# OpenHardware-Initiative/Drone-OA-IREE-ViT-Accelerator

Hardware: AMD Instinct MI355X
Metric: frames/s on ITAViTLSTM int8, 60x90 depth input (higher is better)
Workload: dtype int8+f32; 1 GPU; ITAViTLSTM int8 end-to-end forward (BASELINE config 4): 1024 synthetic 60x90 depth frames per GPU per step, LSTM state carried, velocity all-gather; frames_per_gpu=1024, global_batch=1024, parallelism=dp1, image_dtype=u8, weights=seed-0 synthetic QAT (tests/golden), gather_every=1, gather=none (one GPU), schedule=one stream

## Files before the change

### drone-oa-iree-vit-accelerator_amd/csrc/ita_lstm_head_kernel.h

```cpp
#pragma once
#include <cstddef>
#include "ita_f16x3_kernels.h"

__device__ __forceinline__ size_t ita_lstm_plane_index(int b, int k) {
  return ((size_t)(((b >> 5) * 4 + (k >> 6)) * 4 + ((k >> 4) & 3)) * 64 + ((k >> 3) & 1) * 32 + (b & 31)) * 8 + (k & 7);
}
__device__ __forceinline__ float lstm_sigmoid_fast(float x) {
  return __builtin_amdgcn_rcpf(1.0f + __builtin_amdgcn_exp2f(x * -1.44269504088896341f));
}
__device__ __forceinline__ float lstm_tanh_fast(float x) {
  return 1.0f - 2.0f * __builtin_amdgcn_rcpf(__builtin_amdgcn_exp2f(x * 2.88539008177792681f) + 1.0f);
}

__device__ __forceinline__ f32x16 mfma_f16x3(f32x16 acc, f16x8 wh, f16x8 wl, f16x8 xh, f16x8 xl) {
  acc = __builtin_amdgcn_mfma_f32_32x32x16_f16(wl, xh, acc, 0, 0, 0);
  acc = __builtin_amdgcn_mfma_f32_32x32x16_f16(wh, xl, acc, 0, 0, 0);
  return __builtin_amdgcn_mfma_f32_32x32x16_f16(wh, xh, acc, 0, 0, 0);
}
__device__ __forceinline__ void lstm_cell_fast(float gi, float gf, float gg, float go, float c_prev, float& c, float& h) {
  const float ig = lstm_sigmoid_fast(gi), fg = lstm_sigmoid_fast(gf), cg = lstm_tanh_fast(gg), og = lstm_sigmoid_fast(go);
  c = fmaf(fg, c_prev, ig * cg);
  h = og * lstm_tanh_fast(c);
}
__device__ __forceinline__ void split_f16x4(f32x4 x, f16x4& hi, f16x4& lo) {
#pragma unroll
  for (int j = 0; j < 4; ++j) {
    _Float16 a, b;
    split_f16(x[j], a, b);
    hi[j] = a;
    lo[j] = b;
  }
}
__device__ __forceinline__ f32x4 lstm_l0_extra(float dv, f32x4 q, int h, float& x4) {
  f32x4 x0 = {0.0f, 0.0f, 0.0f, 0.0f};
  x4 = 0.0f;
  if (h == 0) {
    x0 = (f32x4){dv / 10.0f, q.x, q.y, q.z};
    x4 = q.w;
  }
  return x0;
}
template <int NS>
__device__ __forceinline__ f32x4 sum_partials(const f32x4 (&pz)[NS]) {
  f32x4 ps = pz[0];
#pragma unroll
  for (int z = 1; z < NS; ++z) ps += pz[z];
  return ps;
}
__device__ __forceinline__ float lstm_sum4(const float (*part)[16][64], int e, int pl) {
  return ((part[0][e][pl] + part[1][e][pl]) + part[2][e][pl]) + part[3][e][pl];
}
template <class Live>
__device__ __forceinline__ void lstm_fc_rows(const float (*hs)[132], const float (*fw)[128], const float* fc_b, float* vel,
                                             size_t row0, int f0, int B, int tid, Live live) {
  if (tid < 96) {
    const int fr = tid / 3, o = tid - 3 * fr, b = f0 + fr;
    if (b < B && live(b)) {
      float acc = fc_b[o];
      for (int k = 0; k < 128; ++k) acc = fmaf(hs[fr][k], fw[o][k], acc);
      vel[(row0 + b) * 3 + o] = acc;
    }
  }
}

constexpr int ITA_HEAD_CNT_STRIDE = 64;
constexpr unsigned ITA_HEAD_ERR_TIMEOUT = 1;
constexpr unsigned long long ITA_HEAD_SPIN_TICKS = 200000000ull;
__device__ __forceinline__ void ita_store_sc1_f16x4(f16x4 v, __amdgpu_buffer_rsrc_t rsrc, int byte_off) {
  __builtin_amdgcn_raw_buffer_store_b64(__builtin_bit_cast(u32x2, v), rsrc, byte_off, 0, ITA_SC1);
}
__device__ __forceinline__ void ita_gather_h8(float hn, _Float16 (*pub)[32][8], int ef, int eu) {
  _Float16 x, y;
  split_f16(hn, x, y);
  pub[0][ef][eu] = x;
  pub[1][ef][eu] = y;
  __syncthreads();
}
__device__ __forceinline__ void ita_publish_h8(const _Float16 (*pub)[32][8], int r, __amdgpu_buffer_rsrc_t hi, int off_hi,
                                               __amdgpu_buffer_rsrc_t lo, int off_lo) {
  const f16x8 vh = *(const f16x8*)&pub[0][r][0], vl = *(const f16x8*)&pub[1][r][0];
  __builtin_amdgcn_raw_buffer_store_b128(__builtin_bit_cast(u32x4, vh), hi, off_hi, 0, ITA_SC1);
  __builtin_amdgcn_raw_buffer_store_b128(__builtin_bit_cast(u32x4, vl), lo, off_lo, 0, ITA_SC1);
}
__device__ __forceinline__ f16x8 ita_load_sc1_f16x8(__amdgpu_buffer_rsrc_t rsrc, int byte_off) {
  return __builtin_bit_cast(f16x8, __builtin_amdgcn_raw_buffer_load_b128(rsrc, byte_off, 0, ITA_SC1));
}
__device__ __forceinline__ f32x4 ita_load_sc1_f32x4(__amdgpu_buffer_rsrc_t rsrc, int byte_off) {
  return __builtin_bit_cast(f32x4, __builtin_amdgcn_raw_buffer_load_b128(rsrc, byte_off, 0, ITA_SC1));
}
__device__ __forceinline__ unsigned ita_head_arrive(unsigned* cnt, int ft, int tid) {
  asm volatile("s_waitcnt vmcnt(0)" ::: "memory");
  __syncthreads();
  unsigned prev = 0;
  if (tid == 0) prev = __hip_atomic_fetch_add(cnt + ft * ITA_HEAD_CNT_STRIDE, 1u, __ATOMIC_RELAXED, __HIP_MEMORY_SCOPE_AGENT);
// ... 1 lines not shown
}
__device__ __forceinline__ bool ita_head_poll(unsigned* cnt, unsigned target, unsigned* err) {
  const unsigned long long t0 = wall_clock64();
  while (__hip_atomic_load(cnt, __ATOMIC_RELAXED, __HIP_MEMORY_SCOPE_AGENT) < target) {
    if (wall_clock64() - t0 > ITA_HEAD_SPIN_TICKS) {
      __hip_atomic_fetch_or(err, ITA_HEAD_ERR_TIMEOUT, __ATOMIC_RELAXED, __HIP_MEMORY_SCOPE_AGENT);
      return false;
    }
    __builtin_amdgcn_s_sleep(2);
  }
  return true;
}


struct ItaLstmModelArgs {
  const float* part; float inv_fold_scale;
  const _Float16 *w0_hi, *w0_lo; float inv_wscale0;
  const float* bias0;
  const _Float16 *w1_hi, *w1_lo, *w2_hi, *w2_lo;
  float inv_wscale1, inv_wscale2;
  const float *bsum1, *bsum2;
};
struct ItaLstmHeadArgs {
  ItaLstmModelArgs m;
  const float *desvel, *quat;
  const float *h_in, *c_in;
  float *h_out, *c_out;
  size_t lstride;
  _Float16 *p1_hi, *p1_lo, *p2_hi, *p2_lo;
  const float *fc_w, *fc_b; float* vel;
  unsigned *cnt, *err;
  int B;
  const int* slots;
};
static_assert(sizeof(ItaLstmModelArgs) == 104 && offsetof(ItaLstmHeadArgs, desvel) == 104, "kernel-argument layout");

template <int NS>
__global__ __launch_bounds__(256, 2) void ita_lstm_head_kernel(const ItaLstmHeadArgs a) {
  __shared__ __attribute__((aligned(16))) float big[32 * 132 + 32 * 36];
  __shared__ __attribute__((aligned(16))) f16x8 hin[2][2][4][2][64];
  __shared__ __attribute__((aligned(16))) _Float16 pub[2][32][8];
  __shared__ unsigned flag;
  float (*hs)[132] = (float (*)[132])big;
  float (*pt)[36] = (float (*)[36])(big + 32 * 132);
  float (*part)[16][64] = (float (*)[16][64])big;
  const int tid = threadIdx.x, lane = tid & 63, wave = __builtin_amdgcn_readfirstlane(tid >> 6);
  const int ft = blockIdx.x >> 4, ut = blockIdx.x & 15, f0 = ft * 32;
  const int r = lane & 31, h = lane >> 5;
  const int B = a.B;
  const int ef = tid >> 3, eu = tid & 7;
  int rh[4], rb0 = min(f0 + r, B - 1), reb = min(f0 + ef, B - 1);
#pragma unroll
  for (int i = 0; i < 4; ++i) rh[i] = min(f0 + 2 * (4 * wave + i) + h, B - 1);
  if (a.slots) {
#pragma unroll
    for (int i = 0; i < 4; ++i) rh[i] = a.slots[rh[i]];
    rb0 = a.slots[rb0];
    reb = a.slots[reb];
  }

  f32x4 pz[NS];
#pragma unroll
  for (int z = 0; z < NS; ++z)
    pz[z] = *(const f32x4*)(a.m.part + ((size_t)z * B + min(f0 + 8 * wave + (lane >> 3), B - 1)) * 512 + ut * 32 + 4 * (lane & 7));
  f32x4 hv[4];
#pragma unroll
  for (int i = 0; i < 4; ++i) hv[i] = *(const f32x4*)(a.h_in + (size_t)rh[i] * 128 + 4 * r);
  const int b0 = f0 + r, u0 = ut * 8 + 4 * h;
  const size_t sb0 = (size_t)rb0;
  if (wave >= 2) {
    f32x4 hx[2][4][2];
#pragma unroll
    for (int l = 0; l < 2; ++l)
#pragma unroll
      for (int s = 0; s < 4; ++s) {
        const float* src = a.h_in + (l + 1) * a.lstride + sb0 * 128 + 64 * (wave - 2) + 16 * s + 8 * h;
        hx[l][s][0] = *(const f32x4*)src;
        hx[l][s][1] = *(const f32x4*)(src + 4);
      }
    __builtin_amdgcn_sched_barrier(0);
#pragma unroll
    for (int l = 0; l < 2; ++l)
// ... 15 lines not shown
  f32x4 q = {0.0f, 0.0f, 0.0f, 0.0f}, ci0 = {0.0f, 0.0f, 0.0f, 0.0f}, bz[4];
  float dv = 0.0f;
  if (wave == 0) {
    const _Float16* wfr_hi = a.m.w0_hi + ((size_t)ut * 9 * 64 + lane) * 8;
    const _Float16* wfr_lo = a.m.w0_lo + ((size_t)ut * 9 * 64 + lane) * 8;
#pragma unroll
    for (int s = 0; s < 9; ++s) {
      wh[s] = *(const f16x8*)(wfr_hi + s * 512);
      wl[s] = *(const f16x8*)(wfr_lo + s * 512);
    }
    const int bc = min(b0, B - 1);
    q = *(const f32x4*)(a.quat + (size_t)bc * 4);
    dv = a.desvel[bc];
    ci0 = *(const f32x4*)(a.c_in + sb0 * 128 + u0);
#pragma unroll
    for (int gt = 0; gt < 4; ++gt) bz[gt] = *(const f32x4*)(a.m.bias0 + gt * 128 + u0);
  }
  const size_t wo = ((size_t)((ut * 4 + wave) * 4) * 64 + lane) * 8;
  f16x8 w1h[4], w1l[4];
#pragma unroll
  for (int s = 0; s < 4; ++s) {
    w1h[s] = *(const f16x8*)(a.m.w1_hi + wo + 512 * s);
    w1l[s] = *(const f16x8*)(a.m.w1_lo + wo + 512 * s);
  }
  const int eb = f0 + ef, un = ut * 8 + eu;
  const size_t esb = (size_t)reb;
  const float c1_prev = a.c_in[a.lstride + esb * 128 + un], c2_prev = a.c_in[2 * a.lstride + esb * 128 + un];
  float bs1[4], bs2[4];
#pragma unroll
  for (int gt = 0; gt < 4; ++gt) {
    bs1[gt] = a.m.bsum1[gt * 128 + un];
    bs2[gt] = a.m.bsum2[gt * 128 + un];
  }
  __builtin_amdgcn_sched_barrier(0);
  *(f32x4*)&pt[8 * wave + (lane >> 3)][4 * (lane & 7)] = sum_partials(pz);
#pragma unroll
  for (int i = 0; i < 4; ++i) *(f32x4*)&hs[2 * (4 * wave + i) + h][4 * r] = hv[i];
  __syncthreads();

  f32x4 hn0 = {0.0f, 0.0f, 0.0f, 0.0f};
  if (wave == 0) {
    f32x16 acc = {};
    float xlast1;
    const f32x4 xlast0 = lstm_l0_extra(dv, q, h, xlast1);
#pragma unroll
    for (int s = 0; s < 9; ++s) {
      f32x4 x0 = xlast0, x1 = {xlast1, 0.0f, 0.0f, 0.0f};
      if (s < 8) {
        x0 = *(const f32x4*)&hs[r][16 * s + 8 * h];
        x1 = *(const f32x4*)&hs[r][16 * s + 8 * h + 4];
      }
      f16x8 xh, xl;
#pragma unroll
      for (int j = 0; j < 8; ++j) {
        const float x = j < 4 ? x0[j & 3] : x1[j & 3];
        const _Float16 hi = (_Float16)x;
        xh[j] = hi;
        xl[j] = (_Float16)(x - (float)hi);
      }
      acc = mfma_f16x3(acc, wh[s], wl[s], xh, xl);
    }
    f32x4 cn;
#pragma unroll
    for (int q = 0; q < 4; ++q) {
      float g[4];
#pragma unroll
      for (int gt = 0; gt < 4; ++gt)
        g[gt] = (pt[r][gt * 8 + 4 * h + q] * a.m.inv_fold_scale + acc[4 * gt + q] * a.m.inv_wscale0) + bz[gt][q];
      float c, hn;
      lstm_cell_fast(g[0], g[1], g[2], g[3], ci0[q], c, hn);
      cn[q] = c;
      hn0[q] = hn;
    }
    if (b0 < B) *(f32x4*)(a.c_out + sb0 * 128 + u0) = cn;
    f16x4 x_hi, x_lo;
    split_f16x4(hn0, x_hi, x_lo);
    const int o0 = (int)ita_lstm_plane_index(b0, u0) * 2;
    ita_store_sc1_f16x4(x_hi, ita_rsrc(a.p1_hi), o0);
    ita_store_sc1_f16x4(x_lo, ita_rsrc(a.p1_lo), o0);
  }
  (void)ita_head_arrive(a.cnt, ft, tid);
  f16x8 w2h[4], w2l[4];
#pragma unroll
  for (int s = 0; s < 4; ++s) {
    w2h[s] = *(const f16x8*)(a.m.w2_hi + wo + 512 * s);
    w2l[s] = *(const f16x8*)(a.m.w2_lo + wo + 512 * s);
  }

#pragma unroll
  for (int l = 1; l <= 2; ++l) {
    if (tid == 0) flag = ita_head_poll(a.cnt + ft * ITA_HEAD_CNT_STRIDE, 16u * l, a.err) ? 1u : 0u;
    __syncthreads();
    if (!flag) return;
    if (l == 1 && wave == 0 && b0 < B) *(f32x4*)(a.h_out + sb0 * 128 + u0) = hn0;
    f16x8 fah[4], fal[4];
    if (wave < 2) {
      const int ao = (((ft * 4 + wave) * 4) * 64 + lane) * 16;
      const _Float16* ph = l == 1 ? a.p1_hi : a.p2_hi;
      const _Float16* pl = l == 1 ? a.p1_lo : a.p2_lo;
#pragma unroll
      for (int s = 0; s < 4; ++s) {
        fah[s] = ita_load_sc1_f16x8(ita_rsrc(ph), ao + 1024 * s);
        fal[s] = ita_load_sc1_f16x8(ita_rsrc(pl), ao + 1024 * s);
      }
    } else {
#pragma unroll
      for (int s = 0; s < 4; ++s) {
        fah[s] = hin[l - 1][wave - 2][s][0][lane];
        fal[s] = hin[l - 1][wave - 2][s][1][lane];
      }
    }
    f32x16 acc = {};
#pragma unroll
    for (int s = 0; s < 4; ++s) acc = mfma_f16x3(acc, l == 1 ? w1h[s] : w2h[s], l == 1 ? w1l[s] : w2l[s], fah[s], fal[s]);
#pragma unroll
    for (int e = 0; e < 16; ++e) part[wave][e][lane] = acc[e];
    __syncthreads();
    float gsum[4];
    const int pl = ef + 32 * (eu >> 2);
#pragma unroll
    for (int gte = 0; gte < 4; ++gte) gsum[gte] = lstm_sum4(part, 4 * gte + (eu & 3), pl);
    const float iws = l == 1 ? a.m.inv_wscale1 : a.m.inv_wscale2;
    const float* bs = l == 1 ? bs1 : bs2;
    const float gi = gsum[0] * iws + bs[0], gf = gsum[1] * iws + bs[1], gg = gsum[2] * iws + bs[2], go = gsum[3] * iws + bs[3];
    float c, hn;
    lstm_cell_fast(gi, gf, gg, go, l == 1 ? c1_prev : c2_prev, c, hn);
    const size_t so = l * a.lstride + esb * 128 + un;
    if (eb < B) {
      a.c_out[so] = c;
      if (l == 1) a.h_out[so] = hn;
      else
        __builtin_amdgcn_raw_buffer_store_b32(__builtin_bit_cast(unsigned, hn), ita_rsrc(a.h_out), (int)(so * 4), 0, ITA_SC1);
    }
    if (l == 1) {
      ita_gather_h8(hn, pub, ef, eu);
      if (wave == 0 && h == 0) {
        const int o = (int)ita_lstm_plane_index(f0 + r, ut * 8) * 2;
        ita_publish_h8(pub, r, ita_rsrc(a.p2_hi), o, ita_rsrc(a.p2_lo), o);
      }
    }
    const unsigned prev = ita_head_arrive(a.cnt, ft, tid);
    if (tid == 0 && l == 2) flag = prev == 47u ? 1u : 0u;
  }

  __syncthreads();
  if (!flag) return;
  if (tid == 0) __hip_atomic_store(a.cnt + ft * ITA_HEAD_CNT_STRIDE, 0u, __ATOMIC_RELAXED, __HIP_MEMORY_SCOPE_AGENT);
  float (*fw)[128] = (float (*)[128])(big + 32 * 132);
  int fro[4];
#pragma unroll
  for (int i = 0; i < 4; ++i) fro[i] = min(f0 + ((i * 256 + tid) >> 5), B - 1);
  if (a.slots) {
#pragma unroll
    for (int i = 0; i < 4; ++i) fro[i] = a.slots[fro[i]];
  }
  f32x4 hr[4];
#pragma unroll
  for (int i = 0; i < 4; ++i)
    hr[i] = ita_load_sc1_f32x4(ita_rsrc(a.h_out), (int)((2 * a.lstride + (size_t)fro[i] * 128 + 4 * (tid & 31)) * 4));
  const f32x4 wv = *(const f32x4*)(a.fc_w + 4 * min(tid, 95));
#pragma unroll
  for (int i = 0; i < 4; ++i) *(f32x4*)&hs[(i * 256 + tid) >> 5][4 * (tid & 31)] = hr[i];
  if (tid < 96) *(f32x4*)&fw[tid >> 5][4 * (tid & 31)] = wv;
  __syncthreads();
  lstm_fc_rows(hs, fw, a.fc_b, a.vel, 0, f0, B, tid, [](int) { return true; });
}
```

### drone-oa-iree-vit-accelerator_amd/csrc/ita_lstm_seq_kernel.h

```cpp
#pragma once
#include "ita_lstm_head_kernel.h"

constexpr int ITA_SEQ_PLANE = 2 * 4 * 64 * 16;
constexpr int ITA_SEQ_P1 = 0, ITA_SEQ_P2 = 2 * ITA_SEQ_PLANE;
constexpr int ITA_SEQ_H2 = 4 * ITA_SEQ_PLANE;
constexpr int ITA_SEQ_PARITY = ITA_SEQ_H2 + 32 * 128 * 4;
constexpr int ITA_SEQ_TILE = 2 * ITA_SEQ_PARITY;

struct ItaLstmSeqArgs {
  ItaLstmModelArgs m;
  const float *desvel, *quat;
  float *state_h, *state_c;
  const int* lengths; int t0;
  char* ho;
  const float *fc_w, *fc_b; float* vel;
  unsigned *cnt, *err;
  int B, nsteps;
};
static_assert(offsetof(ItaLstmSeqArgs, desvel) == 104, "kernel-argument layout");

__device__ __forceinline__ int ita_seq_plane_off(int r, int k) {
  return ((((k >> 6) * 4 + ((k >> 4) & 3)) * 64 + ((k >> 3) & 1) * 32 + r) * 8 + (k & 7)) * 2;
}

template <int NS>
__global__ __launch_bounds__(256, 1) void ita_lstm_seq_kernel(const ItaLstmSeqArgs a) {
  __shared__ __attribute__((aligned(16))) float big[32 * 132];
  __shared__ __attribute__((aligned(16))) float pt[32][36];
  __shared__ __attribute__((aligned(16))) float fw[3][128];
  __shared__ __attribute__((aligned(16))) _Float16 pub[2][32][8];
  __shared__ __attribute__((aligned(16))) f16x8 w0s[2][9][64];
  __shared__ unsigned flag;
  float (*hs)[132] = (float (*)[132])big;
  float (*acc4)[16][64] = (float (*)[16][64])big;
  const int tid = threadIdx.x, lane = tid & 63, wave = __builtin_amdgcn_readfirstlane(tid >> 6);
  const int ft = blockIdx.x >> 4, ut = blockIdx.x & 15, f0 = ft * 32;
  const int r = lane & 31, h = lane >> 5;
  const int B = a.B;
  unsigned* const cnt = a.cnt + ft * ITA_HEAD_CNT_STRIDE;
  const __amdgpu_buffer_rsrc_t ho = ita_rsrc(a.ho + (size_t)ft * ITA_SEQ_TILE);

  int nt = a.nsteps;
  if (a.lengths) {
    int m = 0;
    for (int i = 0; i < 32; ++i) m = max(m, a.lengths[min(f0 + i, B - 1)]);
    nt = min(nt, max(m - a.t0, 0));
  }
  if (nt <= 0) return;

  const int b0 = f0 + r, u0 = ut * 8 + 4 * h, bc0 = min(b0, B - 1);
  f32x4 c0 = {0.0f, 0.0f, 0.0f, 0.0f}, h0 = {0.0f, 0.0f, 0.0f, 0.0f}, bz[4];
  int len0 = 0;
  if (wave == 0) {
    const _Float16* wfr_hi = a.m.w0_hi + ((size_t)ut * 9 * 64 + lane) * 8;
    const _Float16* wfr_lo = a.m.w0_lo + ((size_t)ut * 9 * 64 + lane) * 8;
#pragma unroll
    for (int s = 0; s < 9; ++s) {
      w0s[0][s][lane] = *(const f16x8*)(wfr_hi + s * 512);
      w0s[1][s][lane] = *(const f16x8*)(wfr_lo + s * 512);
    }
    c0 = *(const f32x4*)(a.state_c + (size_t)bc0 * 128 + u0);
    h0 = *(const f32x4*)(a.state_h + (size_t)bc0 * 128 + u0);
#pragma unroll
    for (int gt = 0; gt < 4; ++gt) bz[gt] = *(const f32x4*)(a.m.bias0 + gt * 128 + u0);
    len0 = b0 < B ? (a.lengths ? a.lengths[b0] - a.t0 : a.nsteps) : 0;
  }
  const size_t wo = ((size_t)((ut * 4 + wave) * 4) * 64 + lane) * 8;
  f16x8 w1h[4], w1l[4], w2h[4], w2l[4];
#pragma unroll
  for (int s = 0; s < 4; ++s) {
    w1h[s] = *(const f16x8*)(a.m.w1_hi + wo + 512 * s);
    w1l[s] = *(const f16x8*)(a.m.w1_lo + wo + 512 * s);
    w2h[s] = *(const f16x8*)(a.m.w2_hi + wo + 512 * s);
    w2l[s] = *(const f16x8*)(a.m.w2_lo + wo + 512 * s);
  }
  const int ef = tid >> 3, eu = tid & 7, eb = f0 + ef, un = ut * 8 + eu, ebc = min(eb, B - 1);
  const size_t lstride = (size_t)B * 128;
  const size_t so1 = lstride + (size_t)ebc * 128 + un, so2 = so1 + lstride;
  float c1 = a.state_c[so1], c2 = a.state_c[so2], h1 = a.state_h[so1], h2 = a.state_h[so2];
  const int lenE = eb < B ? (a.lengths ? a.lengths[eb] - a.t0 : a.nsteps) : 0;
  float bs1[4], bs2[4];
#pragma unroll
  for (int gt = 0; gt < 4; ++gt) {
    bs1[gt] = a.m.bsum1[gt * 128 + un];
    bs2[gt] = a.m.bsum2[gt * 128 + un];
  }
  if (tid < 96) *(f32x4*)&fw[tid >> 5][4 * (tid & 31)] = *(const f32x4*)(a.fc_w + 4 * tid);
  const size_t zstride = (size_t)a.nsteps * B * 512;
  const size_t prow = (size_t)min(f0 + 8 * wave + (lane >> 3), B - 1) * 512 + ut * 32 + 4 * (lane & 7);
  f32x4 ps;
  {
    f32x4 pz[NS];
#pragma unroll
    for (int z = 0; z < NS; ++z) pz[z] = *(const f32x4*)(a.m.part + z * zstride + prow);
    ps = sum_partials(pz);
  }
  f32x4 q = {0.0f, 0.0f, 0.0f, 0.0f};
  float dv = 0.0f;
  if (wave == 0) {
    q = *(const f32x4*)(a.quat + (size_t)bc0 * 4);
    dv = a.desvel[bc0];
  }

  auto publish_h0 = [&](int par) {
    f16x4 x_hi, x_lo;
    split_f16x4(h0, x_hi, x_lo);
    const int o = par * ITA_SEQ_PARITY + ITA_SEQ_P1 + ita_seq_plane_off(r, u0);
    ita_store_sc1_f16x4(x_hi, ho, o);
    ita_store_sc1_f16x4(x_lo, ho, o + ITA_SEQ_PLANE);
  };
  auto publish_h1 = [&](int par) {
    ita_gather_h8(h1, pub, ef, eu);
    if (wave == 0 && h == 0) {
      const int o = par * ITA_SEQ_PARITY + ITA_SEQ_P2 + ita_seq_plane_off(r, ut * 8);
      ita_publish_h8(pub, r, ho, o, ho, o + ITA_SEQ_PLANE);
    }
  };
  auto publish_h2 = [&](int par) {
    __builtin_amdgcn_raw_buffer_store_b32(__builtin_bit_cast(unsigned, h2), ho, par * ITA_SEQ_PARITY + ITA_SEQ_H2 + (ef * 128 + un) * 4,
                                          0, ITA_SC1);
  };
  auto fc_step = [&](int par, int t) {
    f32x4 hr[4];
#pragma unroll
    for (int i = 0; i < 4; ++i)
      hr[i] = ita_load_sc1_f32x4(ho, par * ITA_SEQ_PARITY + ITA_SEQ_H2 + (((i * 256 + tid) >> 5) * 128 + 4 * (tid & 31)) * 4);
#pragma unroll
    for (int i = 0; i < 4; ++i) *(f32x4*)&hs[(i * 256 + tid) >> 5][4 * (tid & 31)] = hr[i];
    __syncthreads();
    lstm_fc_rows(hs, fw, a.fc_b, a.vel, (size_t)t * B, f0, B, tid, [&](int b) { return !a.lengths || a.t0 + t < a.lengths[b]; });
    __syncthreads();
  };

  if (wave == 0) publish_h0(1);
  publish_h1(1);
  publish_h2(1);
  (void)ita_head_arrive(a.cnt, ft, tid);
  if (tid == 0) flag = ita_head_poll(cnt, 16u, a.err) ? 1u : 0u;
  __syncthreads();
  if (!flag) return;

  for (int t = 0; t < nt; ++t) {
    const int par = t & 1, prv = par ^ 1;
    *(f32x4*)&pt[8 * wave + (lane >> 3)][4 * (lane & 7)] = ps;
    f16x8 xh[8], xl[8];
    if (wave == 0) {
#pragma unroll
      for (int s = 0; s < 8; ++s) {
        xh[s] = ita_load_sc1_f16x8(ho, prv * ITA_SEQ_PARITY + ITA_SEQ_P1 + (s * 64 + lane) * 16);
        xl[s] = ita_load_sc1_f16x8(ho, prv * ITA_SEQ_PARITY + ITA_SEQ_P1 + ITA_SEQ_PLANE + (s * 64 + lane) * 16);
      }
    }
    __syncthreads();
    if (wave == 0) {
      f32x16 acc = {};
#pragma unroll
      for (int s = 0; s < 8; ++s) acc = mfma_f16x3(acc, w0s[0][s][lane], w0s[1][s][lane], xh[s], xl[s]);
      {
        float x1;
        const f32x4 x0 = lstm_l0_extra(dv, q, h, x1);
        f16x8 yh, yl;
#pragma unroll
        for (int j = 0; j < 8; ++j) {
          const float x = j < 4 ? x0[j & 3] : (j == 4 ? x1 : 0.0f);
// ... 64 lines not shown
        for (int s = 0; s < 4; ++s)
#pragma unroll
          for (int j = 0; j < 8; ++j) {
            _Float16 hi, lo;
            split_f16(hx[s][j >> 2][j & 3], hi, lo);
            fah[s][j] = hi;
            fal[s][j] = lo;
          }
      }
      f32x16 acc = {};
#pragma unroll
      for (int s = 0; s < 4; ++s) acc = mfma_f16x3(acc, l == 1 ? w1h[s] : w2h[s], l == 1 ? w1l[s] : w2l[s], fah[s], fal[s]);
#pragma unroll
      for (int e = 0; e < 16; ++e) acc4[wave][e][lane] = acc[e];
      __syncthreads();
      float gsum[4];
      const int pl = ef + 32 * (eu >> 2);
#pragma unroll
      for (int gte = 0; gte < 4; ++gte) gsum[gte] = lstm_sum4(acc4, 4 * gte + (eu & 3), pl);
      const float iws = l == 1 ? a.m.inv_wscale1 : a.m.inv_wscale2;
      const float* bs = l == 1 ? bs1 : bs2;
      const float gi = gsum[0] * iws + bs[0], gf = gsum[1] * iws + bs[1], gg = gsum[2] * iws + bs[2], go = gsum[3] * iws + bs[3];
      float c, hn;
      lstm_cell_fast(gi, gf, gg, go, l == 1 ? c1 : c2, c, hn);
      if (t < lenE) {
        if (l == 1) { c1 = c; h1 = hn; }
        else        { c2 = c; h2 = hn; }
      }
      if (l == 1) {
        publish_h1(par);
        (void)ita_head_arrive(a.cnt, ft, tid);
      } else {
        publish_h2(par);
      }
    }
  }

  if (wave == 0 && b0 < B) {
    *(f32x4*)(a.state_c + (size_t)b0 * 128 + u0) = c0;
    *(f32x4*)(a.state_h + (size_t)b0 * 128 + u0) = h0;
  }
  if (eb < B) {
    a.state_c[so1] = c1; a.state_h[so1] = h1;
    a.state_c[so2] = c2; a.state_h[so2] = h2;
  }
  const unsigned prev = ita_head_arrive(a.cnt, ft, tid);
  if (tid == 0) flag = prev == 16u * (2u * nt + 2u) - 1u ? 1u : 0u;
  __syncthreads();
  if (!flag) return;
  if (tid == 0) __hip_atomic_store(cnt, 0u, __ATOMIC_RELAXED, __HIP_MEMORY_SCOPE_AGENT);
  fc_step((nt - 1) & 1, nt - 1);
}
```

### drone-oa-iree-vit-accelerator_amd/csrc/ita_plugin.hip

```cpp
#include <hip/hip_runtime.h>

#include <algorithm>
#include <cstdio>
#include <cstdlib>
#include <cstring>
#include <mutex>
#include <string>
#include <atomic>
#include <thread>
#include <memory>
#include <type_traits>
#include <vector>

#include "../../include/ita_mi355x.h"
#include "../../include/ita_weights.h"
#include "../../include/ita_wire.h"
#include "ita_f16x3_kernels.h"
#include "ita_lstm_head_kernel.h"
#include "ita_lstm_seq_kernel.h"
#include "ita_f32_kernels.h"
#include "ita_int8_kernels.h"
#include "ita_stream_kernel.h"
#include "ita_long_attn_kernel.h"
#include "ita_long_stats_kernel.h"
// ... 86 lines not shown
  operator T*() const { return p; }
};

int launch_tail(int num_cus, int E, const float* wT, const float* bias, const float* x, float* feat, int ld, int B,
                hipStream_t s) {
  if (!wT) return fail(ITA_ERR_BAD_BLOB, "fusion-tail parameters missing from the blob");
  if (E != 64) return fail(ITA_ERR_UNSUPPORTED, "fusion tail is built for E = 64 (ITAViTLSTM)");
  ItaTailArgs a{x, wT, bias, feat, ld, B};
  const int grid = B < 2 * num_cus ? B : 2 * num_cus;
  return launch<ita_tail_kernel<64>, ita_tail_lds_bytes<64>()>(dim3(grid), dim3(256), s, a);
}

int launch_gemm(const float* A, int lda, const float* W, int ldw, const float* bias, float* C, int ldc, int M, int N,
                int K, hipStream_t s) {
  if (N % 64 || K % 32) return fail(ITA_ERR_UNSUPPORTED, "gemm needs N % 64 == 0 and K % 32 == 0");
  ItaGemmArgs g{A, lda, W, ldw, bias, C, ldc, M, N, K};
  return launch<ita_gemm_f32_kernel>(dim3(N / 64, (M + 31) / 32), dim3(256), s, g);
}

}

#include "ita_weights_load.h"

namespace {

struct Workspace {
  int cap = 0;
  int front_cap[ITA_PART_BUFFERS] = {};
  DevBuf<float> bufA, bufB, cat0, cat1, cat2, gates, feat;
  DevBuf<_Float16> x2_hi, x2_lo, c1_hi, c1_lo, c2_hi, c2_lo;
  DevBuf<float> part;
  DevBuf<unsigned> head_sync;
  size_t head_sync_bytes = 0;
  DevBuf<char> seq_ho;
};

struct TailLarge {
  DevBuf<_Float16> hi, lo;
  DevBuf<_Float16> up_hi, up_lo;
  DevBuf<_Float16> ps_hi, ps_lo;
  DevBuf<float> bias;
  float inv_scale = 1.0f;
  int E = 0, CO = 0, nt = 0, nchunk = 0;
};

struct WireSize {
  int H = 0, W = 0;
  DevBuf<int> idx;
  DevBuf<float> coeff;
  ItaWireTables dev{};
  int span[3] = {};
};
constexpr int ITA_WIRE_SIZES = 8;

}

struct ita_context {
  int device = 0;
  int num_cus = 256;
  Weights w;
  Workspace ws;
  bool ws_reserved = false;
  TailLarge tl;
  int tail_mode = 1;
  bool prof = false;
  int prof_max = 0, prof_n = 0;
// ... 15 lines not shown
};

namespace {

std::mutex g_bind_mu;
ita_handle g_bound = nullptr;
int g_bound_layer = 0;
int g_bound_dtype = ITA_DISPATCH_F16;

bool capturing(hipStream_t s) {
  hipStreamCaptureStatus cs = hipStreamCaptureStatusNone;
  return hipStreamIsCapturing(s, &cs) == hipSuccess && cs != hipStreamCaptureStatusNone;
}

int grow_workspace(ita_context* c, int B) {
  c->ws = Workspace{};
  Workspace& ws = c->ws;
  const size_t E = (size_t)c->w.hdr.E, nb = (size_t)B, ntile = (nb + 31) / 32;
  HIPCHK(ws.bufA.alloc(nb * 128 * E));
  HIPCHK(ws.bufB.alloc(nb * 128 * E));
  HIPCHK(ws.feat.alloc(nb * 4608));
  HIPCHK(ws.cat0.alloc(nb * K0P));
  HIPCHK(ws.cat1.alloc(nb * 256));
  HIPCHK(ws.cat2.alloc(nb * 256));
  HIPCHK(ws.gates.alloc(nb * 512));
  HIPCHK(ws.x2_hi.alloc(2 * nb * c->w.ldfold));
  HIPCHK(ws.x2_lo.alloc(2 * nb * c->w.ldfold));
  for (DevBuf<_Float16>* b : {&ws.c1_hi, &ws.c1_lo, &ws.c2_hi, &ws.c2_lo})
    HIPCHK(b->alloc(ntile * 32 * 256));
  HIPCHK(ws.part.alloc(ITA_PART_BUFFERS * (size_t)NSPLIT * nb * 512));
  ws.head_sync_bytes = sizeof(unsigned) * ITA_HEAD_CNT_STRIDE * (1 + ntile);
  HIPCHK(ws.head_sync.alloc(ITA_HEAD_CNT_STRIDE * (1 + ntile)));
  HIPCHK(hipMemset(ws.head_sync, 0, ws.head_sync_bytes));
  HIPCHK(ws.seq_ho.alloc((size_t)ITA_SEQ_TILE * ntile));
  HIPCHK(hipDeviceSynchronize());
  ws.cap = B;
  return ITA_OK;
}

int ensure_workspace(ita_context* c, int B, hipStream_t s) {
  if (B <= c->ws.cap) return ITA_OK;
  if (c->ws_reserved)
    return fail(ITA_ERR_INVALID_ARG, "batch exceeds the workspace pinned by ita_reserve; call ita_reserve(max_batch) again while idle");
  if (capturing(s))
    return fail(ITA_ERR_INVALID_ARG, "the workspace cannot grow inside a stream capture; call ita_reserve first");
  return grow_workspace(c, B);
}

int check(ita_handle h, int batch, bool need_weights = true) {
  if (!h) return fail(ITA_ERR_INVALID_ARG, "null handle");
  if (batch <= 0) return fail(ITA_ERR_INVALID_ARG, "batch must be positive");
  if (need_weights && !h->w.loaded) return fail(ITA_ERR_NO_WEIGHTS, "ita_load_weights has not been called");
  HIPCHK(hipSetDevice(h->device));
  return ITA_OK;
}

int check_layer_io(ita_handle h, int layer, const void* x, const void* y, int batch) {
  if (int rc = check(h, batch)) return rc;
  if (!x || !y || layer < 0 || layer >= h->w.hdr.num_layers) return fail(ITA_ERR_INVALID_ARG, "bad pointer or layer");
  return ITA_OK;
}

ItaMhaArgs mha_args(ita_context* c, int layer, const float* x, float* y, int B, bool fuse, const ita_mha_taps* t) {
  const Layer& L = c->w.layers[layer];
  ItaMhaArgs a{};
  a.x = x; a.y = y;
// ... 983 lines not shown
int ita_get_attn_kind(ita_handle h, int layer, int* kind) {
  if (!h || !h->w.loaded) return fail(ITA_ERR_NO_WEIGHTS, "no weights loaded");
  if (!kind || layer < 0 || layer >= h->w.hdr.num_layers) return fail(ITA_ERR_INVALID_ARG, "bad pointer or layer");
  *kind = h->w.layers[layer].attn_f32 ? ITA_ATTN_F32 : ITA_ATTN_INT8;
  return ITA_OK;
}

int ita_mha_f32(ita_handle h, int layer, const float* x, float* y, int batch, void* stream) {
  if (int rc = check_layer_io(h, layer, x, y, batch)) return rc;
  return launch_attn_f32(h, layer, x, y, batch, false, (hipStream_t)stream);
}

int ita_encoder_layer(ita_handle h, int layer, const float* x, float* y, int batch, void* stream) {
  if (int rc = check_layer_io(h, layer, x, y, batch)) return rc;
  StreamIo io;
  io.x = x; io.y = y;
  return launch_encoder(h, layer, io, batch, (hipStream_t)stream);
}

int ita_debug_encoder_stamps(ita_handle h, int layer, const float* x, const void* image_u8, float* y, int batch,
                             unsigned long long* stamps, void* stream) {
  int rc = check(h, batch);
  if (rc) return rc;
  if ((!x && !image_u8) || !y || !stamps || layer < 0 || layer >= h->w.hdr.num_layers)
    return fail(ITA_ERR_INVALID_ARG, "bad argument");
  if (h->w.layers[layer].attn_f32) return fail(ITA_ERR_UNSUPPORTED, "this layer's attention is float32 (ITAW0003 blob): no stream kernel, no stamps");
  if (image_u8 ? !h->w.layers[layer].simg_tok : !h->w.layers[layer].simg_enc)
    return fail(ITA_ERR_UNSUPPORTED, "this layer does not run on the stream kernel");
  StreamIo io;
  io.x = x; io.y = y; io.stamps = stamps; io.img = image_u8;
  return launch_encoder(h, layer, io, batch, (hipStream_t)stream);
}

#ifdef ITA_UP_STAMP
int ita_debug_tail_up_stamps(unsigned long long* host_dst, int count) {
  if (hipDeviceSynchronize() != hipSuccess) return ITA_ERR_HIP;
  return hipMemcpyFromSymbol(host_dst, HIP_SYMBOL(ita_up_stamp_buf), sizeof(unsigned long long) * (size_t)count) == hipSuccess ? ITA_OK : ITA_ERR_HIP;
}
#endif
int ita_debug_softmax_rows(ita_handle h, const int8_t* logits, uint8_t* probs, int rows, void* stream) {
  int rc = check(h, rows, false);
  if (rc) return rc;
  if (!logits || !probs) return fail(ITA_ERR_INVALID_ARG, "null pointer");
  return launch<ita_softmax_rows_kernel>(dim3((rows + 15) / 16), dim3(64), (hipStream_t)stream, logits, probs, rows);
}

int ita_debug_fast_site_ok(float mult) { return fast_site_ok(mult) ? 1 : 0; }
int ita_debug_fused_site(float mult, int* C, float* K) {
  if (!C || !K) return 0;
  return fused_site(mult, ITA_MAGIC128_F, ITA_FUSED_DMAX, C, K) ? 1 : 0;
}
int ita_debug_fused_check(float mult, int form, int C, float* K) {
  float k = 0.0f;
  const int ok = fused_site_check(mult, form == 1 ? ITA_MAGIC32K_F : form == 2 ? ITA_MAGIC_F : ITA_MAGIC128_F, C, &k) ? 1 : 0;
  if (K) *K = k;
  return ok;
}
int ita_debug_layer_fused(ita_handle h, int layer, unsigned* fused_sites, int* fused, int* C6, float* K6) {
  if (!h || !h->w.loaded) return fail(ITA_ERR_NO_WEIGHTS, "no weights loaded");
  if (!fused_sites || !fused || layer < 0 || layer >= h->w.hdr.num_layers)
    return fail(ITA_ERR_INVALID_ARG, "ita_debug_layer_fused: null output or layer out of range");
  const Layer& L = h->w.layers[layer];
  *fused_sites = L.fused_sites;
  *fused = L.fused ? (L.fused_relu ? 2 : 1) : 0;
  for (int i = 0; i < 6; ++i) {
    if (C6) C6[i] = L.fused_c[i];
// ... 213 lines not shown
      return true;
    };
    if (span_ok(tok_h, OH, 16, ItaTailUpLds::RH) && span_ok(tok_w, OW, 32, ItaTailUpLds::RW)) {
      ItaTailUpArgs u{x, h->tl.up_hi, h->tl.up_lo, h->tl.ps_hi, h->tl.ps_lo, h->tl.bias, h->tl.inv_scale, out, batch, tok_h, tok_w, h->tl.CO};
      const long ntiles = (long)(OW / 32) * (OH / 16) * batch;
      return launch<ita_tail_up_kernel, ItaTailUpLds::TOTAL>(dim3((unsigned)(ntiles < h->num_cus ? ntiles : h->num_cus)), dim3(512), s, u);
    }
  }
  switch (h->tl.nt) {
    case 1: return launch_tail_big<1>(a, s);
    case 2: return launch_tail_big<2>(a, s);
    case 3: return launch_tail_big<3>(a, s);
    default: return launch_tail_big<4>(a, s);
  }
}

static ItaLstmModelArgs lstm_model_args(const ita_context* h, const float* part) {
  const auto& w = h->w;
  ItaLstmModelArgs m;
  m.part = part;          m.inv_fold_scale = w.fold_inv_scale;
  m.w0_hi = w.lw_hi[0];   m.w0_lo = w.lw_lo[0];   m.inv_wscale0 = w.lw_inv_scale[0];
  m.bias0 = w.fold_bias;
  m.w1_hi = w.lw_hi[1];   m.w1_lo = w.lw_lo[1];   m.inv_wscale1 = w.lw_inv_scale[1];
  m.w2_hi = w.lw_hi[2];   m.w2_lo = w.lw_lo[2];   m.inv_wscale2 = w.lw_inv_scale[2];
  m.bsum1 = w.bsum[1];    m.bsum2 = w.bsum[2];
  return m;
}
static dim3 lstm_grid(int B) { return dim3(16 * ((B + 31) / 32)); }

static int launch_lstm_head(ita_context* h, const float* part, const float* desvel, const float* quat, const float* h_in,
                            const float* c_in, float* h_out, float* c_out, size_t lstride, float* vel, int B,
                            const int* slots, hipStream_t s) {
  ItaLstmHeadArgs p{lstm_model_args(h, part), desvel, quat, h_in, c_in, h_out, c_out, lstride,
                    h->ws.c1_hi, h->ws.c1_lo, h->ws.c2_hi, h->ws.c2_lo, h->w.fc_w, h->w.fc_b, vel, h->ws.head_sync + ITA_HEAD_CNT_STRIDE, h->ws.head_sync, B, slots};
  return launch<ita_lstm_head_kernel<NSPLIT>>(lstm_grid(B), dim3(256), s, p);
}

static int launch_lstm_seq(ita_context* h, const float* desvel, const float* quat, float* state_h, float* state_c,
                           const int* lengths, int t0, float* vel, int B, int n, hipStream_t s) {
  ItaLstmSeqArgs p{lstm_model_args(h, h->ws.part), desvel, quat, state_h, state_c, lengths, t0, h->ws.seq_ho,
                   h->w.fc_w, h->w.fc_b, vel, h->ws.head_sync + ITA_HEAD_CNT_STRIDE, h->ws.head_sync, B, n};
  return launch<ita_lstm_seq_kernel<NSPLIT>>(lstm_grid(B), dim3(256), s, p);
}

static int forward_impl(ita_handle h, const void* image, int image_dtype, const float* desvel, const float* quat,
                        const float* h_in, const float* c_in, float* vel, float* h_out, float* c_out, int batch,
                        const ita_forward_taps* taps, void* stream, const int* slots, int state_rows,
                        const float* x2_in = nullptr) {
  int rc = check(h, batch);
  if (rc) return rc;
  if ((!image && !x2_in) || !desvel || !quat || !h_in || !c_in || !vel || !h_out || !c_out)
    return fail(ITA_ERR_INVALID_ARG, "null pointer");
  if (image_dtype != ITA_IMAGE_F32 && image_dtype != ITA_IMAGE_U8) return fail(ITA_ERR_INVALID_ARG, "bad image dtype");
  if (!h->w.dec_w || !h->w.wcat[0] || !h->w.fc_w || (h->w.hdr.has_tail && !h->w.tail_wT))
    return fail(ITA_ERR_BAD_BLOB, "blob holds no decoder / LSTM (/ fusion tail) parameters");
  if (h->w.hdr.has_tail && h->w.hdr.E != 64) return fail(ITA_ERR_UNSUPPORTED, "the fusion tail is built for E = 64 (ITAViTLSTM)");
  if ((rc = ensure_workspace(h, batch, (hipStream_t)stream))) return rc;
  hipStream_t s = (hipStream_t)stream;
  const int B = batch;
  const size_t tokb = sizeof(float) * (size_t)B * 128 * h->w.hdr.E;
  const bool fast = h->tail_mode == 1 && h->w.folded;
  if (slots && !fast) return fail(ITA_ERR_UNSUPPORTED, "slot-indexed state needs tail mode 1");
  const size_t lstride = (size_t)(slots ? state_rows : batch) * 128;
  StageRecorder rec(h, s, true);
  if ((rc = rec.mark())) return rc;
  const bool fused_tok = !x2_in && fuse_tokenizer(h, image_dtype);
  if (slots && !x2_in) {
    const Layer& LL = h->w.layers.back();
// ... 383 lines not shown
```

Baseline: 11.29 million frames/s.

## Distribute final FC head across unit-tile blocks via partial sums

Each of the 16 unit-tile workgroups now computes a 3-output partial dot product over its own 8 hidden units of the last LSTM layer. It publishes these partials to a new fc_part buffer. The last-arriving workgroup then only sums 16 partials per output, instead of reloading the full 32x128 h tile and fc weights and running a 128-long dot product. The sequence kernel gets the same treatment, and optional timestamp instrumentation is added behind a compile flag. This trades an extra small global store per block and a shared barrier for removing the serial tail reload and compute.

```diff
diff --git a/drone-oa-iree-vit-accelerator_amd/csrc/ita_lstm_head_kernel.h b/drone-oa-iree-vit-accelerator_amd/csrc/ita_lstm_head_kernel.h
--- a/drone-oa-iree-vit-accelerator_amd/csrc/ita_lstm_head_kernel.h
+++ b/drone-oa-iree-vit-accelerator_amd/csrc/ita_lstm_head_kernel.h
@@ -50,16 +50,51 @@
 __device__ __forceinline__ float lstm_sum4(const float (*part)[16][64], int e, int pl) {
   return ((part[0][e][pl] + part[1][e][pl]) + part[2][e][pl]) + part[3][e][pl];
 }
+constexpr int ITA_FC_PART_TILE = 16 * 32 * 4;
+__device__ __forceinline__ f32x4 lstm_fc_partial(const float (*hf)[8], int fr, const float (&fcw)[3][8]) {
+  const f32x4 h0 = *(const f32x4*)&hf[fr][0], h1 = *(const f32x4*)&hf[fr][4];
+  f32x4 p = {0.0f, 0.0f, 0.0f, 0.0f};
+#pragma unroll
+  for (int o = 0; o < 3; ++o) {
+    float s = 0.0f;
+#pragma unroll
+    for (int u = 0; u < 8; ++u) s = fmaf(u < 4 ? h0[u & 3] : h1[u & 3], fcw[o][u], s);
+    p[o] = s;
+  }
+  return p;
+}
 template <class Live>
-__device__ __forceinline__ void lstm_fc_rows(const float (*hs)[132], const float (*fw)[128], const float* fc_b, float* vel,
-                                             size_t row0, int f0, int B, int tid, Live live) {
+__device__ __forceinline__ void lstm_fc_sum(__amdgpu_buffer_rsrc_t fp, int byte_off, const float* fc_b, float* vel, size_t row0,
+                                            int f0, int B, int tid, Live live) {
   if (tid < 96) {
     const int fr = tid / 3, o = tid - 3 * fr, b = f0 + fr;
+    float p[16];
+#pragma unroll
+    for (int ut = 0; ut < 16; ++ut)
+      p[ut] = __builtin_bit_cast(float, __builtin_amdgcn_raw_buffer_load_b32(fp, byte_off + ((ut * 32 + fr) * 4 + o) * 4, 0, ITA_SC1));
     if (b < B && live(b)) {
       float acc = fc_b[o];
-      for (int k = 0; k < 128; ++k) acc = fmaf(hs[fr][k], fw[o][k], acc);
+#pragma unroll
+      for (int ut = 0; ut < 16; ++ut) acc += p[ut];
       vel[(row0 + b) * 3 + o] = acc;
     }
+  }
+}
+constexpr int ITA_HEAD_STAMPS = 12, ITA_HEAD_STAMP_WGS = 1024;
+#ifdef ITA_HEAD_STAMP
+__device__ unsigned long long ita_head_stamp_buf[ITA_HEAD_STAMP_WGS * ITA_HEAD_STAMPS];
+constexpr bool ITA_HEAD_STAMPED = true;
+__device__ __forceinline__ void ita_head_stamp_put(int wg, int i) {
+  if (wg < ITA_HEAD_STAMP_WGS) ita_head_stamp_buf[wg * ITA_HEAD_STAMPS + i] = wall_clock64();
+}
+#else
+constexpr bool ITA_HEAD_STAMPED = false;
+__device__ __forceinline__ void ita_head_stamp_put(int, int) {}
+#endif
+template <bool STAMP>
+__device__ __forceinline__ void ita_head_stamp(int i) {
+  if constexpr (STAMP) {
+    if (threadIdx.x == 0) ita_head_stamp_put(blockIdx.x, i);
   }
 }
 
@@ -127,10 +162,11 @@
   unsigned *cnt, *err;
   int B;
   const int* slots;
+  float* fc_part;
 };
 static_assert(sizeof(ItaLstmModelArgs) == 104 && offsetof(ItaLstmHeadArgs, desvel) == 104, "kernel-argument layout");
 
-template <int NS>
+template <int NS, bool STAMP = false>
 __global__ __launch_bounds__(256, 2) void ita_lstm_head_kernel(const ItaLstmHeadArgs a) {
   __shared__ __attribute__((aligned(16))) float big[32 * 132 + 32 * 36];
   __shared__ __attribute__((aligned(16))) f16x8 hin[2][2][4][2][64];
@@ -139,10 +175,12 @@
   float (*hs)[132] = (float (*)[132])big;
   float (*pt)[36] = (float (*)[36])(big + 32 * 132);
   float (*part)[16][64] = (float (*)[16][64])big;
+  float (*hf)[8] = (float (*)[8])pub;
   const int tid = threadIdx.x, lane = tid & 63, wave = __builtin_amdgcn_readfirstlane(tid >> 6);
   const int ft = blockIdx.x >> 4, ut = blockIdx.x & 15, f0 = ft * 32;
   const int r = lane & 31, h = lane >> 5;
   const int B = a.B;
+  ita_head_stamp<STAMP>(0);
   const int ef = tid >> 3, eu = tid & 7;
   int rh[4], rb0 = min(f0 + r, B - 1), reb = min(f0 + ef, B - 1);
 #pragma unroll
@@ -224,11 +262,17 @@
     bs1[gt] = a.m.bsum1[gt * 128 + un];
     bs2[gt] = a.m.bsum2[gt * 128 + un];
   }
+  float fcw[3][8];
+#pragma unroll
+  for (int o = 0; o < 3; ++o)
+#pragma unroll
+    for (int u = 0; u < 8; ++u) fcw[o][u] = a.fc_w[o * 128 + ut * 8 + u];
   __builtin_amdgcn_sched_barrier(0);
   *(f32x4*)&pt[8 * wave + (lane >> 3)][4 * (lane & 7)] = sum_partials(pz);
 #pragma unroll
   for (int i = 0; i < 4; ++i) *(f32x4*)&hs[2 * (4 * wave + i) + h][4 * r] = hv[i];
   __syncthreads();
+  ita_head_stamp<STAMP>(1);
 
   f32x4 hn0 = {0.0f, 0.0f, 0.0f, 0.0f};
   if (wave == 0) {
@@ -272,6 +316,7 @@
     ita_store_sc1_f16x4(x_lo, ita_rsrc(a.p1_lo), o0);
   }
   (void)ita_head_arrive(a.cnt, ft, tid);
+  ita_head_stamp<STAMP>(2);
   f16x8 w2h[4], w2l[4];
 #pragma unroll
   for (int s = 0; s < 4; ++s) {
@@ -284,6 +329,7 @@
     if (tid == 0) flag = ita_head_poll(a.cnt + ft * ITA_HEAD_CNT_STRIDE, 16u * l, a.err) ? 1u : 0u;
     __syncthreads();
     if (!flag) return;
+    ita_head_stamp<STAMP>(2 * l + 1);
     if (l == 1 && wave == 0 && b0 < B) *(f32x4*)(a.h_out + sb0 * 128 + u0) = hn0;
     f16x8 fah[4], fal[4];
     if (wave < 2) {
@@ -320,9 +366,7 @@
     const size_t so = l * a.lstride + esb * 128 + un;
     if (eb < B) {
       a.c_out[so] = c;
-      if (l == 1) a.h_out[so] = hn;
-      else
-        __builtin_amdgcn_raw_buffer_store_b32(__builtin_bit_cast(unsigned, hn), ita_rsrc(a.h_out), (int)(so * 4), 0, ITA_SC1);
+      a.h_out[so] = hn;
     }
     if (l == 1) {
       ita_gather_h8(hn, pub, ef, eu);
@@ -330,30 +374,24 @@
         const int o = (int)ita_lstm_plane_index(f0 + r, ut * 8) * 2;
         ita_publish_h8(pub, r, ita_rsrc(a.p2_hi), o, ita_rsrc(a.p2_lo), o);
       }
+    } else {
+      hf[ef][eu] = hn;
+      __syncthreads();
+      if (wave == 0 && h == 0)
+        __builtin_amdgcn_raw_buffer_store_b128(__builtin_bit_cast(u32x4, lstm_fc_partial(hf, r, fcw)),
+                                               ita_rsrc(a.fc_part + (size_t)ft * ITA_FC_PART_TILE), (ut * 32 + r) * 16, 0, ITA_SC1);
     }
     const unsigned prev = ita_head_arrive(a.cnt, ft, tid);
     if (tid == 0 && l == 2) flag = prev == 47u ? 1u : 0u;
+    ita_head_stamp<STAMP>(2 * l + 2);
   }
 
   __syncthreads();
   if (!flag) return;
   if (tid == 0) __hip_atomic_store(a.cnt + ft * ITA_HEAD_CNT_STRIDE, 0u, __ATOMIC_RELAXED, __HIP_MEMORY_SCOPE_AGENT);
-  float (*fw)[128] = (float (*)[128])(big + 32 * 132);
-  int fro[4];
-#pragma unroll
-  for (int i = 0; i < 4; ++i) fro[i] = min(f0 + ((i * 256 + tid) >> 5), B - 1);
-  if (a.slots) {
-#pragma unroll
-    for (int i = 0; i < 4; ++i) fro[i] = a.slots[fro[i]];
-  }
-  f32x4 hr[4];
-#pragma unroll
-  for (int i = 0; i < 4; ++i)
-    hr[i] = ita_load_sc1_f32x4(ita_rsrc(a.h_out), (int)((2 * a.lstride + (size_t)fro[i] * 128 + 4 * (tid & 31)) * 4));
-  const f32x4 wv = *(const f32x4*)(a.fc_w + 4 * min(tid, 95));
-#pragma unroll
-  for (int i = 0; i < 4; ++i) *(f32x4*)&hs[(i * 256 + tid) >> 5][4 * (tid & 31)] = hr[i];
-  if (tid < 96) *(f32x4*)&fw[tid >> 5][4 * (tid & 31)] = wv;
-  __syncthreads();
-  lstm_fc_rows(hs, fw, a.fc_b, a.vel, 0, f0, B, tid, [](int) { return true; });
-}
+  lstm_fc_sum(ita_rsrc(a.fc_part + (size_t)ft * ITA_FC_PART_TILE), 0, a.fc_b, a.vel, 0, f0, B, tid, [](int) { return true; });
+  if constexpr (STAMP) {
+    asm volatile("s_waitcnt vmcnt(0)" ::: "memory");
+    ita_head_stamp<STAMP>(8);
+  }
+}
diff --git a/drone-oa-iree-vit-accelerator_amd/csrc/ita_lstm_seq_kernel.h b/drone-oa-iree-vit-accelerator_amd/csrc/ita_lstm_seq_kernel.h
--- a/drone-oa-iree-vit-accelerator_amd/csrc/ita_lstm_seq_kernel.h
+++ b/drone-oa-iree-vit-accelerator_amd/csrc/ita_lstm_seq_kernel.h
@@ -4,7 +4,8 @@
 constexpr int ITA_SEQ_PLANE = 2 * 4 * 64 * 16;
 constexpr int ITA_SEQ_P1 = 0, ITA_SEQ_P2 = 2 * ITA_SEQ_PLANE;
 constexpr int ITA_SEQ_H2 = 4 * ITA_SEQ_PLANE;
-constexpr int ITA_SEQ_PARITY = ITA_SEQ_H2 + 32 * 128 * 4;
+constexpr int ITA_SEQ_FCP = ITA_SEQ_H2 + 32 * 128 * 4;
+constexpr int ITA_SEQ_PARITY = ITA_SEQ_FCP + ITA_FC_PART_TILE * 4;
 constexpr int ITA_SEQ_TILE = 2 * ITA_SEQ_PARITY;
 
 struct ItaLstmSeqArgs {
@@ -25,14 +26,14 @@
 
 template <int NS>
 __global__ __launch_bounds__(256, 1) void ita_lstm_seq_kernel(const ItaLstmSeqArgs a) {
-  __shared__ __attribute__((aligned(16))) float big[32 * 132];
+  __shared__ __attribute__((aligned(16))) float big[4 * 16 * 64];
   __shared__ __attribute__((aligned(16))) float pt[32][36];
-  __shared__ __attribute__((aligned(16))) float fw[3][128];
+  __shared__ float fws[3][8];
   __shared__ __attribute__((aligned(16))) _Float16 pub[2][32][8];
   __shared__ __attribute__((aligned(16))) f16x8 w0s[2][9][64];
   __shared__ unsigned flag;
-  float (*hs)[132] = (float (*)[132])big;
   float (*acc4)[16][64] = (float (*)[16][64])big;
+  float (*hf)[8] = (float (*)[8])pub;
   const int tid = threadIdx.x, lane = tid & 63, wave = __builtin_amdgcn_readfirstlane(tid >> 6);
   const int ft = blockIdx.x >> 4, ut = blockIdx.x & 15, f0 = ft * 32;
   const int r = lane & 31, h = lane >> 5;
@@ -85,7 +86,7 @@
     bs1[gt] = a.m.bsum1[gt * 128 + un];
     bs2[gt] = a.m.bsum2[gt * 128 + un];
   }
-  if (tid < 96) *(f32x4*)&fw[tid >> 5][4 * (tid & 31)] = *(const f32x4*)(a.fc_w + 4 * tid);
+  if (tid < 24) fws[tid >> 3][tid & 7] = a.fc_w[(tid >> 3) * 128 + ut * 8 + (tid & 7)];
   const size_t zstride = (size_t)a.nsteps * B * 512;
   const size_t prow = (size_t)min(f0 + 8 * wave + (lane >> 3), B - 1) * 512 + ut * 32 + 4 * (lane & 7);
   f32x4 ps;
@@ -121,15 +122,8 @@
                                           0, ITA_SC1);
   };
   auto fc_step = [&](int par, int t) {
-    f32x4 hr[4];
-#pragma unroll
-    for (int i = 0; i < 4; ++i)
-      hr[i] = ita_load_sc1_f32x4(ho, par * ITA_SEQ_PARITY + ITA_SEQ_H2 + (((i * 256 + tid) >> 5) * 128 + 4 * (tid & 31)) * 4);
-#pragma unroll
-    for (int i = 0; i < 4; ++i) *(f32x4*)&hs[(i * 256 + tid) >> 5][4 * (tid & 31)] = hr[i];
-    __syncthreads();
-    lstm_fc_rows(hs, fw, a.fc_b, a.vel, (size_t)t * B, f0, B, tid, [&](int b) { return !a.lengths || a.t0 + t < a.lengths[b]; });
-    __syncthreads();
+    lstm_fc_sum(ho, par * ITA_SEQ_PARITY + ITA_SEQ_FCP, a.fc_b, a.vel, (size_t)t * B, f0, B, tid,
+                [&](int b) { return !a.lengths || a.t0 + t < a.lengths[b]; });
   };
 
   if (wave == 0) publish_h0(1);
@@ -260,6 +254,17 @@
         (void)ita_head_arrive(a.cnt, ft, tid);
       } else {
         publish_h2(par);
+        hf[ef][eu] = h2;
+        __syncthreads();
+        if (wave == 0 && h == 0) {
+          float fcw[3][8];
+#pragma unroll
+          for (int o = 0; o < 3; ++o)
+#pragma unroll
+            for (int u = 0; u < 8; ++u) fcw[o][u] = fws[o][u];
+          __builtin_amdgcn_raw_buffer_store_b128(__builtin_bit_cast(u32x4, lstm_fc_partial(hf, r, fcw)), ho,
+                                                 par * ITA_SEQ_PARITY + ITA_SEQ_FCP + (ut * 32 + r) * 16, 0, ITA_SC1);
+        }
       }
     }
   }
diff --git a/drone-oa-iree-vit-accelerator_amd/csrc/ita_plugin.hip b/drone-oa-iree-vit-accelerator_amd/csrc/ita_plugin.hip
--- a/drone-oa-iree-vit-accelerator_amd/csrc/ita_plugin.hip
+++ b/drone-oa-iree-vit-accelerator_amd/csrc/ita_plugin.hip
@@ -142,6 +142,7 @@
   DevBuf<float> part;
   DevBuf<unsigned> head_sync;
   size_t head_sync_bytes = 0;
+  DevBuf<float> fc_part;
   DevBuf<char> seq_ho;
 };
 
@@ -223,6 +224,7 @@
   ws.head_sync_bytes = sizeof(unsigned) * ITA_HEAD_CNT_STRIDE * (1 + ntile);
   HIPCHK(ws.head_sync.alloc(ITA_HEAD_CNT_STRIDE * (1 + ntile)));
   HIPCHK(hipMemset(ws.head_sync, 0, ws.head_sync_bytes));
+  HIPCHK(ws.fc_part.alloc((size_t)ITA_FC_PART_TILE * ntile));
   HIPCHK(ws.seq_ho.alloc((size_t)ITA_SEQ_TILE * ntile));
   HIPCHK(hipDeviceSynchronize());
   ws.cap = B;
@@ -1272,6 +1274,12 @@
   return launch_encoder(h, layer, io, batch, (hipStream_t)stream);
 }
 
+#ifdef ITA_HEAD_STAMP
+int ita_debug_head_stamps(unsigned long long* host_dst, int count) {
+  if (!host_dst || count <= 0 || count > ITA_HEAD_STAMP_WGS * ITA_HEAD_STAMPS) return fail(ITA_ERR_INVALID_ARG, "bad stamp buffer");
+  return hipMemcpyFromSymbol(host_dst, HIP_SYMBOL(ita_head_stamp_buf), sizeof(unsigned long long) * (size_t)count) == hipSuccess ? ITA_OK : ITA_ERR_HIP;
+}
+#endif
 #ifdef ITA_UP_STAMP
 int ita_debug_tail_up_stamps(unsigned long long* host_dst, int count) {
   if (hipDeviceSynchronize() != hipSuccess) return ITA_ERR_HIP;
@@ -1551,8 +1559,9 @@
                             const float* c_in, float* h_out, float* c_out, size_t lstride, float* vel, int B,
                             const int* slots, hipStream_t s) {
   ItaLstmHeadArgs p{lstm_model_args(h, part), desvel, quat, h_in, c_in, h_out, c_out, lstride,
-                    h->ws.c1_hi, h->ws.c1_lo, h->ws.c2_hi, h->ws.c2_lo, h->w.fc_w, h->w.fc_b, vel, h->ws.head_sync + ITA_HEAD_CNT_STRIDE, h->ws.head_sync, B, slots};
-  return launch<ita_lstm_head_kernel<NSPLIT>>(lstm_grid(B), dim3(256), s, p);
+                    h->ws.c1_hi, h->ws.c1_lo, h->ws.c2_hi, h->ws.c2_lo, h->w.fc_w, h->w.fc_b, vel, h->ws.head_sync + ITA_HEAD_CNT_STRIDE, h->ws.head_sync, B, slots,
+                    h->ws.fc_part};
+  return launch<ita_lstm_head_kernel<NSPLIT, ITA_HEAD_STAMPED>>(lstm_grid(B), dim3(256), s, p);
 }
 
 static int launch_lstm_seq(ita_context* h, const float* desvel, const float* quat, float* state_h, float* state_c,
```

Result: no change. 11.28 million frames/s (median of 2 runs) (-0.1%).
